# tangxyw/RecAlgorithm

Hardware: NVIDIA H100
Metric: ctr_fwd_bwd_samples_per_sec (higher is better)
Workload: dtype f32

## Files before the change

### recalgorithm_b200/csrc/c_api.cu

```cuda
#include <stdarg.h>
#include <string.h>

#include <atomic>

#include "ctr_common.cuh"

namespace ctr {
static thread_local char g_err[512] = "";
static std::atomic<long long> g_launches{0};

void set_error(const char* fmt, ...) {
  va_list ap;
  va_start(ap, fmt);
  vsnprintf(g_err, sizeof(g_err), fmt, ap);
  va_end(ap);
}
void count_launch(int n) { g_launches.fetch_add(n, std::memory_order_relaxed); }

int sm_count() {
  static int cached[64] = {0};
  int dev = 0;
  if (cudaGetDevice(&dev) != cudaSuccess || dev < 0 || dev >= 64) return 132;
  if (cached[dev] == 0) {
    int n = 0;
    if (cudaDeviceGetAttribute(&n, cudaDevAttrMultiProcessorCount, dev) != cudaSuccess || n <= 0) n = 132;
    cached[dev] = n;
  }
  return cached[dev];
}
}

extern "C" {
const char* ctr_last_error(void) { return ctr::g_err; }
int ctr_version(void) { return 1; }
int64_t ctr_kernel_launches(void) { return ctr::g_launches.load(); }

int ctr_enable_peer_access(int peer_device) {
  int dev = 0;
  CTR_CUDA(cudaGetDevice(&dev));
  if (peer_device == dev) return CTR_OK;
  int can = 0;
  CTR_CUDA(cudaDeviceCanAccessPeer(&can, dev, peer_device));
  if (!can) {
    ctr::set_error("ctr_enable_peer_access: device %d cannot access device %d over P2P", dev, peer_device);
    return CTR_ERR_UNSUPPORTED;
  }
  cudaError_t e = cudaDeviceEnablePeerAccess(peer_device, 0);
  if (e == cudaErrorPeerAccessAlreadyEnabled) { cudaGetLastError(); return CTR_OK; }
  if (e != cudaSuccess) {
    ctr::set_error("cudaDeviceEnablePeerAccess(%d) failed: %s", peer_device, cudaGetErrorString(e));
    return CTR_ERR_CUDA;
  }
  return CTR_OK;
}

int ctr_peer_alloc(int64_t bytes, void** ptr) {
  CTR_REQUIRE(ptr != nullptr && bytes > 0, "ctr_peer_alloc: bad arguments");
  CTR_CUDA(cudaMalloc(ptr, (size_t)bytes));
  return CTR_OK;
}
int ctr_peer_free(void* ptr) {
  if (ptr) CTR_CUDA(cudaFree(ptr));
  return CTR_OK;
}
int ctr_ipc_export(void* ptr, unsigned char* handle64) {
  CTR_REQUIRE(ptr && handle64, "ctr_ipc_export: null argument");
  static_assert(sizeof(cudaIpcMemHandle_t) == 64, "CUDA IPC handle is 64 bytes");
  cudaIpcMemHandle_t h;
  CTR_CUDA(cudaIpcGetMemHandle(&h, ptr));
  memcpy(handle64, &h, 64);
  return CTR_OK;
}
int ctr_ipc_import(const unsigned char* handle64, void** ptr) {
  CTR_REQUIRE(ptr && handle64, "ctr_ipc_import: null argument");
  cudaIpcMemHandle_t h;
  memcpy(&h, handle64, 64);
  CTR_CUDA(cudaIpcOpenMemHandle(ptr, h, cudaIpcMemLazyEnablePeerAccess));
  return CTR_OK;
}
int ctr_ipc_close(void* ptr) {
  if (ptr) CTR_CUDA(cudaIpcCloseMemHandle(ptr));
  return CTR_OK;
}

int ctr_device_info(int* sm_count, int* cc_major, int* cc_minor) {
  int dev = 0;
  CTR_CUDA(cudaGetDevice(&dev));
  int v = 0;
  if (sm_count) { CTR_CUDA(cudaDeviceGetAttribute(&v, cudaDevAttrMultiProcessorCount, dev)); *sm_count = v; }
  if (cc_major) { CTR_CUDA(cudaDeviceGetAttribute(&v, cudaDevAttrComputeCapabilityMajor, dev)); *cc_major = v; }
  if (cc_minor) { CTR_CUDA(cudaDeviceGetAttribute(&v, cudaDevAttrComputeCapabilityMinor, dev)); *cc_minor = v; }
  return CTR_OK;
}
}
```

### recalgorithm_b200/csrc/ctr_common.cuh

```cuda
#pragma once
#include <cuda_runtime.h>
#include <stdint.h>
#include <stdio.h>

#include <type_traits>

#include "../../include/ctr_b200.h"

namespace ctr {

void set_error(const char* fmt, ...);
void count_launch(int n = 1);
int sm_count();

#define CTR_REQUIRE(cond, ...)                                   \
  do {                                                           \
    if (!(cond)) {                                               \
      ctr::set_error(__VA_ARGS__);                               \
      return CTR_ERR_INVALID_ARG;                                \
    }                                                            \
  } while (0)

#define CTR_UNSUPPORTED(cond, ...)                               \
  do {                                                           \
    if (cond) {                                                  \
      ctr::set_error(__VA_ARGS__);                               \
      return CTR_ERR_UNSUPPORTED;                                \
    }                                                            \
  } while (0)

#define CTR_CHECK_LAUNCH(name)                                                   \
  do {                                                                           \
    cudaError_t e__ = cudaGetLastError();                                        \
    if (e__ != cudaSuccess) {                                                    \
      ctr::set_error("%s: launch failed: %s", name, cudaGetErrorString(e__));    \
      return CTR_ERR_CUDA;                                                       \
    }                                                                            \
    ctr::count_launch();                                                         \
  } while (0)

#define CTR_CUDA(call)                                                           \
  do {                                                                           \
    cudaError_t e__ = (call);                                                    \
    if (e__ != cudaSuccess) {                                                    \
      ctr::set_error("%s failed: %s", #call, cudaGetErrorString(e__));           \
      return CTR_ERR_CUDA;                                                       \
    }                                                                            \
  } while (0)

__device__ __forceinline__ float warp_sum(float v) {
#pragma unroll
  for (int o = 16; o > 0; o >>= 1) v += __shfl_xor_sync(0xffffffffu, v, o);
  return v;
}

__device__ __forceinline__ float4 ldg_stream_f4(const float4* p) {
  float4 r;
  asm volatile("ld.global.nc.L1::no_allocate.v4.f32 {%0,%1,%2,%3}, [%4];"
               : "=f"(r.x), "=f"(r.y), "=f"(r.z), "=f"(r.w) : "l"(p));
  return r;
}
__device__ __forceinline__ void stg_stream_f4(float4* p, const float4& v) {
  asm volatile("st.global.cs.v4.f32 [%0], {%1,%2,%3,%4};" ::"l"(p), "f"(v.x), "f"(v.y), "f"(v.z), "f"(v.w)
               : "memory");
}
__device__ __forceinline__ long long ldg_stream_i64(const long long* p) {
  long long r;
  asm volatile("ld.global.nc.L1::no_allocate.s64 %0, [%1];" : "=l"(r) : "l"(p));
  return r;
}

static inline cudaStream_t as_stream(void* s) { return reinterpret_cast<cudaStream_t>(s); }
static inline bool aligned16(const void* p) { return (reinterpret_cast<uintptr_t>(p) & 15u) == 0; }

static inline int capped_grid(long long need, long long cap) { return (int)(need < cap ? need : cap); }

template <class... P, class... A>
int launch(const char* what, void (*k)(P...), dim3 grid, dim3 block, size_t smem, cudaStream_t st, const A&... args) {
  if (smem > 48 * 1024) CTR_CUDA(cudaFuncSetAttribute(k, cudaFuncAttributeMaxDynamicSharedMemorySize, (int)smem));
  k<<<grid, block, smem, st>>>(args...);
  CTR_CHECK_LAUNCH(what);
  return CTR_OK;
}

template <int MAX_PER_SM = 0, class... P, class... A>
int launch_resident(const char* what, void (*k)(P...), long long need, int block, size_t smem, cudaStream_t st,
                    const A&... args) {
  if (smem > 48 * 1024) CTR_CUDA(cudaFuncSetAttribute(k, cudaFuncAttributeMaxDynamicSharedMemorySize, (int)smem));
  int per_sm = 0;
  if (cudaOccupancyMaxActiveBlocksPerMultiprocessor(&per_sm, k, block, smem) != cudaSuccess || per_sm < 1) per_sm = 1;
  if (MAX_PER_SM > 0 && per_sm > MAX_PER_SM) per_sm = MAX_PER_SM;
  k<<<capped_grid(need, (long long)per_sm * sm_count()), block, smem, st>>>(args...);
  CTR_CHECK_LAUNCH(what);
  return CTR_OK;
}

template <int... Vs, class F>
int with_const(int v, F&& f) {
  int rc = CTR_OK;
  const bool hit = ((v == Vs && ((rc = f(std::integral_constant<int, Vs>{})), true)) || ...);
  if (!hit) {
    set_error("no kernel instantiation for %d", v);
    return CTR_ERR_INVALID_ARG;
  }
  return rc;
}
template <class F>
int with_lpr(int64_t D, F&& f) {
  return with_const<1, 2, 4, 8, 16, 32>((int)(D / 4), f);
}

}
```

### recalgorithm_b200/csrc/embed_fm2.cu

```cuda
#include "ctr_common.cuh"

namespace ctr {

__device__ __forceinline__ float4 f4_zero() { return make_float4(0.f, 0.f, 0.f, 0.f); }

struct PeerTables {
  const float4* base[8];
  int G, logG;
};

__device__ __forceinline__ long long load_id(const long long* p) { return ldg_stream_i64(p); }
__device__ __forceinline__ long long load_id(const int* p) {
  int r;
  asm volatile("ld.global.nc.L1::no_allocate.s32 %0, [%1];" : "=r"(r) : "l"(p));
  return (long long)r;
}
__device__ __forceinline__ float4 ld_peer_f4(const float4* p) {
  float4 r;
  asm volatile("ld.global.v4.f32 {%0,%1,%2,%3}, [%4];" : "=f"(r.x), "=f"(r.y), "=f"(r.z), "=f"(r.w) : "l"(p));
  return r;
}

template <int LPR, bool SH, int MINB, bool BI = false, typename IdT = long long, bool LIN = false, bool SEQ = false>
__global__ void __launch_bounds__(256, MINB)
embed_fm2_fwd_kernel(const float4* __restrict__ table, const PeerTables peers, const long long* __restrict__ row_off,
                     const IdT* __restrict__ ids, int B, int F, float4* __restrict__ tile,
                     float* __restrict__ fm2, long long* __restrict__ ids64_out,
                     const float4* __restrict__ wlin, float* __restrict__ lin) {
  constexpr int RPW = 32 / LPR;
  constexpr int UB = LPR < 8 ? LPR : 8;
  const unsigned full = 0xffffffffu;
  const int lane = threadIdx.x & 31;
  const int sub = lane / LPR;
  const int c = lane % LPR;
  const int warp0 = (blockIdx.x * blockDim.x + threadIdx.x) >> 5;
  const int nwarps = (gridDim.x * blockDim.x) >> 5;

  for (int b = warp0; b < B; b += nwarps) {
    float4 S = f4_zero(), Q = f4_zero();
    float lin_acc = 0.f;
    for (int f0 = 0; f0 < F; f0 += 32) {
      const int nf = min(32, F - f0);
      long long row = -1;
      if (lane < nf) {
        const long long id = load_id(ids + (size_t)b * F + f0 + lane);
        const long long lo = __ldg(row_off + (SEQ ? 0 : f0 + lane)), hi = __ldg(row_off + (SEQ ? 1 : f0 + lane + 1));
        row = (id >= 0 && id < hi - lo) ? lo + id : -1;
        if (sizeof(IdT) == 4 && ids64_out != nullptr) ids64_out[(size_t)b * F + f0 + lane] = id;
      }
#pragma unroll
      for (int it0 = 0; it0 < LPR; it0 += UB) {
        if (it0 * RPW >= nf) break;
        float4 v[UB];
        bool in[UB];
#pragma unroll
        for (int u = 0; u < UB; ++u) {
          const int fs = (it0 + u) * RPW + sub;
          const long long r = __shfl_sync(full, row, fs);
          in[u] = fs < nf;
          v[u] = f4_zero();
          if (in[u] && r >= 0) {
            if (SH) v[u] = ld_peer_f4(peers.base[r & (peers.G - 1)] + (size_t)(r >> peers.logG) * LPR + c);
            else v[u] = ldg_stream_f4(table + (size_t)r * LPR + c);
          }
        }
#pragma unroll
        for (int u = 0; u < UB; ++u) {
          S.x += v[u].x; S.y += v[u].y; S.z += v[u].z; S.w += v[u].w;
          Q.x = __fadd_rn(Q.x, __fmul_rn(v[u].x, v[u].x)); Q.y = __fadd_rn(Q.y, __fmul_rn(v[u].y, v[u].y));
          Q.z = __fadd_rn(Q.z, __fmul_rn(v[u].z, v[u].z)); Q.w = __fadd_rn(Q.w, __fmul_rn(v[u].w, v[u].w));
          if (tile != nullptr && in[u]) {
            const int fs = (it0 + u) * RPW + sub;
            stg_stream_f4(tile + ((size_t)b * F + f0 + fs) * LPR + c, v[u]);
          }
          if (LIN && in[u]) {
            const float4 w = __ldg(wlin + (size_t)(f0 + (it0 + u) * RPW + sub) * LPR + c);
            lin_acc += v[u].x * w.x + v[u].y * w.y + v[u].z * w.z + v[u].w * w.w;
          }
        }
      }
    }
    if (LIN) {
      lin_acc = warp_sum(lin_acc);
      if (lane == 0) lin[b] = lin_acc;
    }
    if (fm2 != nullptr) {
#pragma unroll
      for (int o = LPR; o < 32; o <<= 1) {
        S.x += __shfl_xor_sync(full, S.x, o); S.y += __shfl_xor_sync(full, S.y, o);
        S.z += __shfl_xor_sync(full, S.z, o); S.w += __shfl_xor_sync(full, S.w, o);
        Q.x += __shfl_xor_sync(full, Q.x, o); Q.y += __shfl_xor_sync(full, Q.y, o);
        Q.z += __shfl_xor_sync(full, Q.z, o); Q.w += __shfl_xor_sync(full, Q.w, o);
      }
      if (BI) {
        if (lane < LPR) {
          float4 r;
          r.x = 0.5f * __fsub_rn(__fmul_rn(S.x, S.x), Q.x); r.y = 0.5f * __fsub_rn(__fmul_rn(S.y, S.y), Q.y);
          r.z = 0.5f * __fsub_rn(__fmul_rn(S.z, S.z), Q.z); r.w = 0.5f * __fsub_rn(__fmul_rn(S.w, S.w), Q.w);
          reinterpret_cast<float4*>(fm2)[(size_t)b * LPR + c] = r;
        }
        continue;
      }
      float p = 0.5f * __fsub_rn(__fmul_rn(S.x, S.x), Q.x) + 0.5f * __fsub_rn(__fmul_rn(S.y, S.y), Q.y) +
                0.5f * __fsub_rn(__fmul_rn(S.z, S.z), Q.z) + 0.5f * __fsub_rn(__fmul_rn(S.w, S.w), Q.w);
#pragma unroll
      for (int o = 1; o < LPR; o <<= 1) p += __shfl_xor_sync(full, p, o);
      if (lane == 0) fm2[b] = p;
    }
  }
}

template <int LPR, int HOLD, bool BI = false>
__global__ void __launch_bounds__(256)
embed_fm2_bwd_kernel(const float4* __restrict__ tile, const float4* __restrict__ d_tile,
                     const float* __restrict__ d_fm2, int B, int F, float4* __restrict__ row_grads) {
  const unsigned full = 0xffffffffu;
  const int lane = threadIdx.x & 31;
  const int warp0 = (blockIdx.x * blockDim.x + threadIdx.x) >> 5;
  const int nwarps = (gridDim.x * blockDim.x) >> 5;
  const int n4 = F * LPR;

  for (int b = warp0; b < B; b += nwarps) {
    const float4* e_row = tile + (size_t)b * n4;
    float4* o_row = row_grads + (size_t)b * n4;
    const float4* dt_row = d_tile ? d_tile + (size_t)b * n4 : nullptr;
    float4 g4;
    if (BI) {
      g4 = __ldg(reinterpret_cast<const float4*>(d_fm2) + (size_t)b * LPR + lane % LPR);
    } else {
      const float g = d_fm2 ? __ldg(d_fm2 + b) : 0.f;
      g4 = make_float4(g, g, g, g);
    }
    float4 S = f4_zero();
    if (HOLD > 0) {
      constexpr int H = HOLD > 0 ? HOLD : 1;
      float4 e[H];
#pragma unroll
      for (int k = 0; k < H; ++k) {
        const int j = k * 32 + lane;
        e[k] = f4_zero();
        if (j < n4) e[k] = ldg_stream_f4(e_row + j);
      }
      float4 dt[H];
#pragma unroll
      for (int k = 0; k < H; ++k) {
        const int j = k * 32 + lane;
        dt[k] = f4_zero();
        if (dt_row != nullptr && j < n4) dt[k] = ldg_stream_f4(dt_row + j);
      }
#pragma unroll
      for (int k = 0; k < H; ++k) { S.x += e[k].x; S.y += e[k].y; S.z += e[k].z; S.w += e[k].w; }
#pragma unroll
      for (int o = LPR; o < 32; o <<= 1) {
        S.x += __shfl_xor_sync(full, S.x, o); S.y += __shfl_xor_sync(full, S.y, o);
        S.z += __shfl_xor_sync(full, S.z, o); S.w += __shfl_xor_sync(full, S.w, o);
      }
#pragma unroll
      for (int k = 0; k < H; ++k) {
        const int j = k * 32 + lane;
        if (j < n4) {
          float4 r;
          r.x = dt[k].x + g4.x * (S.x - e[k].x); r.y = dt[k].y + g4.y * (S.y - e[k].y);
          r.z = dt[k].z + g4.z * (S.z - e[k].z); r.w = dt[k].w + g4.w * (S.w - e[k].w);
          stg_stream_f4(o_row + j, r);
        }
      }
    } else {
      for (int j = lane; j < n4; j += 32) {
        const float4 v = __ldg(e_row + j);
        S.x += v.x; S.y += v.y; S.z += v.z; S.w += v.w;
      }
#pragma unroll
      for (int o = LPR; o < 32; o <<= 1) {
        S.x += __shfl_xor_sync(full, S.x, o); S.y += __shfl_xor_sync(full, S.y, o);
        S.z += __shfl_xor_sync(full, S.z, o); S.w += __shfl_xor_sync(full, S.w, o);
      }
      for (int j = lane; j < n4; j += 32) {
        const float4 v = __ldg(e_row + j);
        float4 r = dt_row ? ldg_stream_f4(dt_row + j) : f4_zero();
        r.x += g4.x * (S.x - v.x); r.y += g4.y * (S.y - v.y); r.z += g4.z * (S.z - v.z); r.w += g4.w * (S.w - v.w);
        stg_stream_f4(o_row + j, r);
      }
    }
  }
}

template <int LPR, int HOLD>
__global__ void __launch_bounds__(256, 2)
embed_fm2_lin_bwd_kernel(const float4* __restrict__ tile, const float4* __restrict__ wlin, const float* __restrict__ d_fm2,
                         const float* __restrict__ d_lin, int B, int F, float4* __restrict__ row_grads,
                         float4* __restrict__ d_wlin) {
  extern __shared__ float4 s_lin[];
  const unsigned full = 0xffffffffu;
  const int lane = threadIdx.x & 31;
  const int warp0 = (blockIdx.x * blockDim.x + threadIdx.x) >> 5;
  const int nwarps = (gridDim.x * blockDim.x) >> 5;
  const int n4 = F * LPR;
  float4* s_w = s_lin;
  float4* s_dw = s_lin + n4;
  for (int j = threadIdx.x; j < n4; j += blockDim.x) { s_w[j] = __ldg(wlin + j); s_dw[j] = f4_zero(); }
  __syncthreads();
  float4 acc[HOLD];
#pragma unroll
  for (int k = 0; k < HOLD; ++k) acc[k] = f4_zero();
  for (int b = warp0; b < B; b += nwarps) {
    const float4* e_row = tile + (size_t)b * n4;
    float4* o_row = row_grads + (size_t)b * n4;
    const float g = d_fm2 ? __ldg(d_fm2 + b) : 0.f;
    const float gl = d_lin ? __ldg(d_lin + b) : 0.f;
    float4 e[HOLD];
#pragma unroll
    for (int k = 0; k < HOLD; ++k) {
      const int j = k * 32 + lane;
      e[k] = f4_zero();
      if (j < n4) e[k] = ldg_stream_f4(e_row + j);
    }
    float4 S = f4_zero();
#pragma unroll
    for (int k = 0; k < HOLD; ++k) { S.x += e[k].x; S.y += e[k].y; S.z += e[k].z; S.w += e[k].w; }
#pragma unroll
    for (int o = LPR; o < 32; o <<= 1) {
      S.x += __shfl_xor_sync(full, S.x, o); S.y += __shfl_xor_sync(full, S.y, o);
      S.z += __shfl_xor_sync(full, S.z, o); S.w += __shfl_xor_sync(full, S.w, o);
    }
#pragma unroll
    for (int k = 0; k < HOLD; ++k) {
      const int j = k * 32 + lane;
      if (j < n4) {
        const float4 w = s_w[j];
        float4 r;
        r.x = gl * w.x + g * (S.x - e[k].x); r.y = gl * w.y + g * (S.y - e[k].y);
        r.z = gl * w.z + g * (S.z - e[k].z); r.w = gl * w.w + g * (S.w - e[k].w);
        stg_stream_f4(o_row + j, r);
        acc[k].x += gl * e[k].x; acc[k].y += gl * e[k].y; acc[k].z += gl * e[k].z; acc[k].w += gl * e[k].w;
      }
    }
  }
#pragma unroll
  for (int k = 0; k < HOLD; ++k) {
    const int j = k * 32 + lane;
    if (j < n4) {
      atomicAdd(&s_dw[j].x, acc[k].x); atomicAdd(&s_dw[j].y, acc[k].y);
      atomicAdd(&s_dw[j].z, acc[k].z); atomicAdd(&s_dw[j].w, acc[k].w);
    }
  }
  __syncthreads();
  for (int j = threadIdx.x; j < n4; j += blockDim.x) atomicAdd(d_wlin + j, s_dw[j]);
}

template <int LPR>
__global__ void __launch_bounds__(256)
embed_scatter_add_kernel(float4* __restrict__ grad_table, const long long* __restrict__ row_off,
                         const long long* __restrict__ ids, const float4* __restrict__ row_grads, int B, int F) {
  const size_t total = (size_t)B * F * LPR;
  for (size_t t = (size_t)blockIdx.x * blockDim.x + threadIdx.x; t < total; t += (size_t)gridDim.x * blockDim.x) {
    const int c = (int)(t % LPR);
    const size_t bf = t / LPR;
    const int f = (int)(bf % F);
    const long long id = __ldg(ids + bf);
    const long long lo = __ldg(row_off + f), hi = __ldg(row_off + f + 1);
    if (id >= 0 && id < hi - lo) {
      const float4 g = ldg_stream_f4(row_grads + t);
      atomicAdd(grad_table + (size_t)(lo + id) * LPR + c, g);
    }
  }
}

__global__ void __launch_bounds__(256)
bag_lookup_fwd_kernel(const float* __restrict__ table, long long V, int D, const long long* __restrict__ ids,
                      const long long* __restrict__ offsets, int B, float* __restrict__ out, long long out_stride,
                      int G) {
  const int tid = blockIdx.x * blockDim.x + threadIdx.x;
  const int gl = threadIdx.x % G;
  const int nthreads = gridDim.x * blockDim.x;
  for (int b = tid / G; b < B; b += nthreads / G) {
    const long long s = __ldg(offsets + b), e = __ldg(offsets + b + 1);
    float acc[8];
#pragma unroll
    for (int k = 0; k < 8; ++k) acc[k] = 0.f;
    int n = 0;
    for (long long i = s; i < e; ++i) {
      const long long id = __ldg(ids + i);
      if (id >= 0 && id < V) {
        ++n;
#pragma unroll
        for (int k = 0; k < 8; ++k) {
          const int dd = k * G + gl;
          if (dd < D) acc[k] += __ldg(table + (size_t)id * D + dd);
        }
      }
    }
#pragma unroll
    for (int k = 0; k < 8; ++k) {
      const int dd = k * G + gl;
      if (dd < D) out[(size_t)b * out_stride + dd] = n > 0 ? acc[k] / (float)n : 0.f;
    }
  }
}

__global__ void __launch_bounds__(256)
bag_lookup_bwd_kernel(const float* __restrict__ d_out, long long out_stride, long long V, int D,
                      const long long* __restrict__ ids, const long long* __restrict__ offsets, int B,
                      float* __restrict__ row_grads, int G) {
  const int tid = blockIdx.x * blockDim.x + threadIdx.x;
  const int gl = threadIdx.x % G;
  const int nthreads = gridDim.x * blockDim.x;
  for (int b = tid / G; b < B; b += nthreads / G) {
    const long long s = __ldg(offsets + b), e = __ldg(offsets + b + 1);
    int n = 0;
    for (long long i = s; i < e; ++i) {
      const long long id = __ldg(ids + i);
      n += (id >= 0 && id < V);
    }
    for (long long i = s; i < e; ++i) {
      const long long id = __ldg(ids + i);
      const bool ok = id >= 0 && id < V;
      for (int dd = gl; dd < D; dd += G) {
        const float g = __ldg(d_out + (size_t)b * out_stride + dd);
        row_grads[(size_t)i * D + dd] = ok ? g / (float)n : 0.f;
      }
    }
  }
}

__global__ void __launch_bounds__(256)
first_order_fwd_kernel(const float* __restrict__ w, const long long* __restrict__ row_off,
                       const long long* __restrict__ ids, int B, int F, float bias, float* __restrict__ out) {
  const int lane = threadIdx.x & 31;
  const int warp0 = (blockIdx.x * blockDim.x + threadIdx.x) >> 5;
  const int nwarps = (gridDim.x * blockDim.x) >> 5;
  for (int b = warp0; b < B; b += nwarps) {
    float acc = 0.f;
    for (int f = lane; f < F; f += 32) {
      const long long id = ldg_stream_i64(ids + (size_t)b * F + f);
      const long long lo = __ldg(row_off + f), hi = __ldg(row_off + f + 1);
      if (id >= 0 && id < hi - lo) acc += __ldg(w + lo + id);
    }
    acc = warp_sum(acc);
    if (lane == 0) out[b] = acc + bias;
  }
}

template <int LPR, typename IdT>
static int launch_fwd(const float* table, const PeerTables* peers, const int64_t* off, const IdT* ids, int64_t B,
                      int64_t F, float* tile, float* fm2, int64_t* ids64_out, cudaStream_t st) {
  PeerTables none = {};
  const PeerTables& pt = peers ? *peers : none;
  auto go = [&](auto k) {
    return launch_resident("ctr_embed_fm2_fwd", k, (B + 7) / 8, 256, 0, st, reinterpret_cast<const float4*>(table), pt,
                           reinterpret_cast<const long long*>(off), ids, (int)B, (int)F, reinterpret_cast<float4*>(tile), fm2,
                           reinterpret_cast<long long*>(ids64_out), nullptr, nullptr);
  };
  return peers != nullptr ? go(embed_fm2_fwd_kernel<LPR, true, 1, false, IdT>) : go(embed_fm2_fwd_kernel<LPR, false, 4, false, IdT>);
}

template <int LPR, int HOLD, bool BI = false>
static int launch_bwd(const float* tile, const float* d_tile, const float* d_fm2, int64_t B, int64_t F,
                      float* row_grads, cudaStream_t st) {
  return launch_resident("ctr_embed_fm2_bwd", embed_fm2_bwd_kernel<LPR, HOLD, BI>, (B + 7) / 8, 256, 0, st,
                         reinterpret_cast<const float4*>(tile), reinterpret_cast<const float4*>(d_tile), d_fm2, (int)B, (int)F,
                         reinterpret_cast<float4*>(row_grads));
}

template <int LPR, bool BI = false>
static int dispatch_bwd(const float* tile, const float* d_tile, const float* d_fm2, int64_t B, int64_t F,
                        float* row_grads, cudaStream_t st) {
  const int64_t per_lane = (F * LPR + 31) / 32;
  if (per_lane <= 4) return launch_bwd<LPR, 4, BI>(tile, d_tile, d_fm2, B, F, row_grads, st);
  if (per_lane <= 8) return launch_bwd<LPR, 8, BI>(tile, d_tile, d_fm2, B, F, row_grads, st);
  if (per_lane <= 12) return launch_bwd<LPR, 12, BI>(tile, d_tile, d_fm2, B, F, row_grads, st);
  return launch_bwd<LPR, 0, BI>(tile, d_tile, d_fm2, B, F, row_grads, st);
}

template <int LPR>
static int launch_fwd_bi(const float* table, const int64_t* off, const int64_t* ids, int64_t B, int64_t F, float* tile,
                         float* bi, cudaStream_t st) {
  return launch_resident("ctr_embed_bi_fwd", embed_fm2_fwd_kernel<LPR, false, 4, true>, (B + 7) / 8, 256, 0, st,
                         reinterpret_cast<const float4*>(table), PeerTables{}, reinterpret_cast<const long long*>(off),
                         reinterpret_cast<const long long*>(ids), (int)B, (int)F, reinterpret_cast<float4*>(tile), bi, nullptr,
                         nullptr, nullptr);
}

static int check_bfd(const char* fn, int64_t B, int64_t F, int64_t D) {
  CTR_REQUIRE(B >= 0 && F >= 1 && D >= 1, "%s: bad sizes B=%lld F=%lld D=%lld", fn, (long long)B, (long long)F,
              (long long)D);
  CTR_REQUIRE(B <= 0x7fffffffLL / 8 && F <= 65536, "%s: B=%lld / F=%lld too large", fn, (long long)B, (long long)F);
  CTR_UNSUPPORTED(D % 4 != 0 || D > 128 || (D & (D - 1)) != 0,
                  "%s: D=%lld unsupported by the fused 128-bit path (need a power of two in 4..128); "
                  "use ctr_bag_lookup_* for other widths", fn, (long long)D);
  return CTR_OK;
}

template <typename IdT>
static int dispatch_fwd(const float* table, const PeerTables* peers, const int64_t* off, const IdT* ids, int64_t B,
                        int64_t F, int64_t D, float* tile, float* fm2, int64_t* ids64_out, cudaStream_t st) {
  return with_lpr(D, [&](auto LPR) { return launch_fwd<LPR>(table, peers, off, ids, B, F, tile, fm2, ids64_out, st); });
}

static int fill_peers(const char* fn, PeerTables& peers, const float* const* shard_ptrs, int64_t G) {
  CTR_REQUIRE(G >= 1 && G <= 8 && (G & (G - 1)) == 0, "%s: G=%lld must be a power of two <= 8", fn, (long long)G);
  peers = PeerTables{};
  peers.G = (int)G;
  while ((1 << peers.logG) < G) ++peers.logG;
  for (int r = 0; r < G; ++r) {
    CTR_REQUIRE(shard_ptrs[r] != nullptr && aligned16(shard_ptrs[r]), "%s: shard %d null/unaligned", fn, r);
    peers.base[r] = reinterpret_cast<const float4*>(shard_ptrs[r]);
  }
  return CTR_OK;
}

}

using namespace ctr;

extern "C" int ctr_embed_fm2_fwd(const float* table, const int64_t* field_row_offset, const int64_t* ids,
                                 int64_t B, int64_t F, int64_t D, float* tile, float* fm2, void* stream) {
  int rc = check_bfd("ctr_embed_fm2_fwd", B, F, D);
  if (rc) return rc;
  CTR_REQUIRE(table && field_row_offset && ids, "ctr_embed_fm2_fwd: null table/field_row_offset/ids");
  CTR_REQUIRE(tile || fm2, "ctr_embed_fm2_fwd: both outputs are NULL");
  CTR_REQUIRE(aligned16(table) && aligned16(tile), "ctr_embed_fm2_fwd: table and tile must be 16-byte aligned");
  if (B == 0) return CTR_OK;
  cudaStream_t st = as_stream(stream);
  return dispatch_fwd(table, nullptr, field_row_offset, reinterpret_cast<const long long*>(ids), B, F, D, tile, fm2, nullptr, st);
}

extern "C" int ctr_embed_fm2_fwd_ids32(const float* table, const int64_t* field_row_offset, const int32_t* ids, int64_t B,
                                       int64_t F, int64_t D, float* tile, float* fm2, int64_t* ids64_out, void* stream) {
  int rc = check_bfd("ctr_embed_fm2_fwd_ids32", B, F, D);
  if (rc) return rc;
  CTR_REQUIRE(table && field_row_offset && ids, "ctr_embed_fm2_fwd_ids32: null table/field_row_offset/ids");
  CTR_REQUIRE(tile || fm2, "ctr_embed_fm2_fwd_ids32: both outputs are NULL");
  CTR_REQUIRE(aligned16(table) && aligned16(tile), "ctr_embed_fm2_fwd_ids32: table and tile must be 16-byte aligned");
  if (B == 0) return CTR_OK;
  return dispatch_fwd(table, nullptr, field_row_offset, reinterpret_cast<const int*>(ids), B, F, D, tile, fm2, ids64_out,
                      as_stream(stream));
}

extern "C" int ctr_embed_fm2_fwd_sharded(const float* const* shard_ptrs, int64_t G, const int64_t* field_row_offset,
                                         const int64_t* ids, int64_t B, int64_t F, int64_t D, float* tile, float* fm2,
                                         void* stream) {
  int rc = check_bfd("ctr_embed_fm2_fwd_sharded", B, F, D);
  if (rc) return rc;
  CTR_REQUIRE(shard_ptrs && field_row_offset && ids, "ctr_embed_fm2_fwd_sharded: null shard_ptrs/field_row_offset/ids");
  CTR_REQUIRE(tile || fm2, "ctr_embed_fm2_fwd_sharded: both outputs are NULL");
  PeerTables peers;
  rc = fill_peers("ctr_embed_fm2_fwd_sharded", peers, shard_ptrs, G);
  if (rc) return rc;
  CTR_REQUIRE(aligned16(tile), "ctr_embed_fm2_fwd_sharded: tile must be 16-byte aligned");
  if (B == 0) return CTR_OK;
  return dispatch_fwd(nullptr, &peers, field_row_offset, reinterpret_cast<const long long*>(ids), B, F, D, tile, fm2, nullptr,
                      as_stream(stream));
}

extern "C" int ctr_embed_fm2_fwd_sharded_ids32(const float* const* shard_ptrs, int64_t G, const int64_t* field_row_offset,
                                               const int32_t* ids, int64_t B, int64_t F, int64_t D, float* tile, float* fm2,
                                               int64_t* ids64_out, void* stream) {
  int rc = check_bfd("ctr_embed_fm2_fwd_sharded_ids32", B, F, D);
  if (rc) return rc;
  CTR_REQUIRE(shard_ptrs && field_row_offset && ids, "ctr_embed_fm2_fwd_sharded_ids32: null shard_ptrs/field_row_offset/ids");
  CTR_REQUIRE(tile || fm2, "ctr_embed_fm2_fwd_sharded_ids32: both outputs are NULL");
  PeerTables peers;
  rc = fill_peers("ctr_embed_fm2_fwd_sharded_ids32", peers, shard_ptrs, G);
  if (rc) return rc;
  CTR_REQUIRE(aligned16(tile), "ctr_embed_fm2_fwd_sharded_ids32: tile must be 16-byte aligned");
  if (B == 0) return CTR_OK;
  return dispatch_fwd(nullptr, &peers, field_row_offset, reinterpret_cast<const int*>(ids), B, F, D, tile, fm2, ids64_out,
                      as_stream(stream));
}

extern "C" int ctr_embed_fm2_bwd(const float* tile, const float* d_tile, const float* d_fm2, int64_t B, int64_t F,
                                 int64_t D, float* row_grads, void* stream) {
  int rc = check_bfd("ctr_embed_fm2_bwd", B, F, D);
  if (rc) return rc;
  CTR_REQUIRE(tile && row_grads, "ctr_embed_fm2_bwd: null tile/row_grads");
  CTR_REQUIRE(aligned16(tile) && aligned16(d_tile) && aligned16(row_grads),
              "ctr_embed_fm2_bwd: tile, d_tile and row_grads must be 16-byte aligned");
  if (B == 0) return CTR_OK;
  cudaStream_t st = as_stream(stream);
  return with_lpr(D, [&](auto LPR) { return dispatch_bwd<LPR>(tile, d_tile, d_fm2, B, F, row_grads, st); });
}

extern "C" int ctr_embed_scatter_add(float* grad_table, const int64_t* field_row_offset, const int64_t* ids,
                                     const float* row_grads, int64_t B, int64_t F, int64_t D, void* stream) {
  int rc = check_bfd("ctr_embed_scatter_add", B, F, D);
  if (rc) return rc;
  CTR_REQUIRE(grad_table && field_row_offset && ids && row_grads, "ctr_embed_scatter_add: null argument");
  CTR_REQUIRE(aligned16(grad_table) && aligned16(row_grads), "ctr_embed_scatter_add: buffers must be 16-byte aligned");
  if (B == 0) return CTR_OK;
  cudaStream_t st = as_stream(stream);
  const long long total = (long long)B * F * (D / 4);
  const int grid = capped_grid((total + 255) / 256, (long long)sm_count() * 16);
  return with_lpr(D, [&](auto LPR) {
    return launch("ctr_embed_scatter_add", embed_scatter_add_kernel<LPR>, grid, 256, 0, st, reinterpret_cast<float4*>(grad_table),
                  reinterpret_cast<const long long*>(field_row_offset), reinterpret_cast<const long long*>(ids),
                  reinterpret_cast<const float4*>(row_grads), (int)B, (int)F);
  });
}

static int bag_group(int64_t D) {
  int G = 1;
  while (G < D && G < 32) G <<= 1;
  return G;
}

extern "C" int ctr_bag_lookup_fwd(const float* table, int64_t V, int64_t D, const int64_t* ids,
                                  const int64_t* offsets, int64_t B, float* out, int64_t out_stride, void* stream) {
  CTR_REQUIRE(table && offsets && out, "ctr_bag_lookup_fwd: null argument");
  CTR_REQUIRE(B >= 0 && V >= 0 && D >= 1 && out_stride >= D, "ctr_bag_lookup_fwd: bad sizes");
  CTR_UNSUPPORTED(D > 256, "ctr_bag_lookup_fwd: D=%lld > 256", (long long)D);
  if (B == 0) return CTR_OK;
  const int G = bag_group(D);
  return launch("ctr_bag_lookup_fwd", bag_lookup_fwd_kernel, capped_grid(((long long)B * G + 255) / 256, (long long)sm_count() * 16),
                256, 0, as_stream(stream), table, V, (int)D, reinterpret_cast<const long long*>(ids),
                reinterpret_cast<const long long*>(offsets), (int)B, out, out_stride, G);
}

extern "C" int ctr_bag_lookup_bwd(const float* d_out, int64_t out_stride, int64_t V, int64_t D, const int64_t* ids,
                                  const int64_t* offsets, int64_t B, float* row_grads, void* stream) {
  CTR_REQUIRE(d_out && offsets, "ctr_bag_lookup_bwd: null argument");
  CTR_REQUIRE(B >= 0 && V >= 0 && D >= 1 && out_stride >= D, "ctr_bag_lookup_bwd: bad sizes");
  CTR_UNSUPPORTED(D > 256, "ctr_bag_lookup_bwd: D=%lld > 256", (long long)D);
  if (B == 0) return CTR_OK;
  const int G = bag_group(D);
  return launch("ctr_bag_lookup_bwd", bag_lookup_bwd_kernel, capped_grid(((long long)B * G + 255) / 256, (long long)sm_count() * 16),
                256, 0, as_stream(stream), d_out, out_stride, V, (int)D, reinterpret_cast<const long long*>(ids),
                reinterpret_cast<const long long*>(offsets), (int)B, row_grads, G);
}

extern "C" int ctr_first_order_fwd(const float* w, const int64_t* field_row_offset, const int64_t* ids, int64_t B,
                                   int64_t F, float bias, float* out, void* stream) {
  CTR_REQUIRE(w && field_row_offset && ids && out, "ctr_first_order_fwd: null argument");
  CTR_REQUIRE(B >= 0 && F >= 1 && B <= 0x7fffffffLL / 8 && F <= 65536, "ctr_first_order_fwd: bad sizes");
  if (B == 0) return CTR_OK;
  return launch("ctr_first_order_fwd", first_order_fwd_kernel, capped_grid((B + 7) / 8, (long long)sm_count() * 8), 256, 0,
                as_stream(stream), w, reinterpret_cast<const long long*>(field_row_offset), reinterpret_cast<const long long*>(ids),
                (int)B, (int)F, bias, out);
}

extern "C" int ctr_embed_bi_fwd(const float* table, const int64_t* field_row_offset, const int64_t* ids, int64_t B, int64_t F,
                                int64_t D, float* tile, float* bi, void* stream) {
  int rc = check_bfd("ctr_embed_bi_fwd", B, F, D);
  if (rc) return rc;
  CTR_REQUIRE(table && field_row_offset && ids && bi, "ctr_embed_bi_fwd: null table/field_row_offset/ids/bi");
  CTR_REQUIRE(aligned16(table) && aligned16(tile) && aligned16(bi), "ctr_embed_bi_fwd: table, tile and bi must be 16-byte aligned");
  if (B == 0) return CTR_OK;
  cudaStream_t st = as_stream(stream);
  return with_lpr(D, [&](auto LPR) { return launch_fwd_bi<LPR>(table, field_row_offset, ids, B, F, tile, bi, st); });
}

extern "C" int ctr_embed_bi_bwd(const float* tile, const float* d_tile, const float* d_bi, int64_t B, int64_t F, int64_t D,
                                float* row_grads, void* stream) {
  int rc = check_bfd("ctr_embed_bi_bwd", B, F, D);
  if (rc) return rc;
  CTR_REQUIRE(tile && d_bi && row_grads, "ctr_embed_bi_bwd: null tile/d_bi/row_grads");
  CTR_REQUIRE(aligned16(tile) && aligned16(d_tile) && aligned16(d_bi) && aligned16(row_grads),
              "ctr_embed_bi_bwd: tile, d_tile, d_bi and row_grads must be 16-byte aligned");
  if (B == 0) return CTR_OK;
  cudaStream_t st = as_stream(stream);
  return with_lpr(D, [&](auto LPR) { return dispatch_bwd<LPR, true>(tile, d_tile, d_bi, B, F, row_grads, st); });
}

template <int LPR, typename IdT>
static int launch_fwd_lin(const float* table, const PeerTables* peers, const int64_t* off, const IdT* ids, int64_t B, int64_t F,
                          float* tile, float* fm2, int64_t* ids64_out, const float* wlin, float* lin, cudaStream_t st) {
  auto go = [&](auto k, const float4* tb, const PeerTables& pt) {
    return launch_resident("ctr_embed_fm2_lin_fwd", k, (B + 7) / 8, 256, 0, st, tb, pt, reinterpret_cast<const long long*>(off),
                           ids, (int)B, (int)F, reinterpret_cast<float4*>(tile), fm2, reinterpret_cast<long long*>(ids64_out),
                           reinterpret_cast<const float4*>(wlin), lin);
  };
  if (peers != nullptr) return go(embed_fm2_fwd_kernel<LPR, true, 1, false, IdT, true>, nullptr, *peers);
  return go(embed_fm2_fwd_kernel<LPR, false, 3, false, IdT, true>, reinterpret_cast<const float4*>(table), PeerTables{});
}

template <typename IdT>
static int dispatch_fwd_lin(const float* table, const PeerTables* peers, const int64_t* off, const IdT* ids, int64_t B, int64_t F,
                            int64_t D, float* tile, float* fm2, int64_t* ids64_out, const float* wlin, float* lin, cudaStream_t st) {
  return with_lpr(D, [&](auto LPR) { return launch_fwd_lin<LPR>(table, peers, off, ids, B, F, tile, fm2, ids64_out, wlin, lin, st); });
}

extern "C" int ctr_embed_fm2_lin_fwd(const float* table, const int64_t* field_row_offset, const void* ids, int ids_are_int32,
                                     int64_t B, int64_t F, int64_t D, const float* wlin, float* tile, float* fm2, float* lin,
                                     int64_t* ids64_out, void* stream) {
  int rc = check_bfd("ctr_embed_fm2_lin_fwd", B, F, D);
  if (rc) return rc;
  CTR_REQUIRE(table && field_row_offset && ids && wlin && lin, "ctr_embed_fm2_lin_fwd: null table/field_row_offset/ids/wlin/lin");
  CTR_REQUIRE(aligned16(table) && aligned16(tile) && aligned16(wlin), "ctr_embed_fm2_lin_fwd: table, tile and wlin must be 16-byte aligned");
  if (B == 0) return CTR_OK;
  cudaStream_t st = as_stream(stream);
  if (ids_are_int32)
    return dispatch_fwd_lin(table, nullptr, field_row_offset, reinterpret_cast<const int*>(ids), B, F, D, tile, fm2, ids64_out, wlin, lin, st);
  return dispatch_fwd_lin(table, nullptr, field_row_offset, reinterpret_cast<const long long*>(ids), B, F, D, tile, fm2, nullptr, wlin, lin, st);
}

extern "C" int ctr_embed_fm2_lin_fwd_sharded(const float* const* shard_ptrs, int64_t G, const int64_t* field_row_offset,
                                             const void* ids, int ids_are_int32, int64_t B, int64_t F, int64_t D, const float* wlin,
                                             float* tile, float* fm2, float* lin, int64_t* ids64_out, void* stream) {
  int rc = check_bfd("ctr_embed_fm2_lin_fwd_sharded", B, F, D);
  if (rc) return rc;
  CTR_REQUIRE(shard_ptrs && field_row_offset && ids && wlin && lin, "ctr_embed_fm2_lin_fwd_sharded: null argument");
  PeerTables peers;
  rc = fill_peers("ctr_embed_fm2_lin_fwd_sharded", peers, shard_ptrs, G);
  if (rc) return rc;
  CTR_REQUIRE(aligned16(tile) && aligned16(wlin), "ctr_embed_fm2_lin_fwd_sharded: tile and wlin must be 16-byte aligned");
  if (B == 0) return CTR_OK;
  cudaStream_t st = as_stream(stream);
  if (ids_are_int32)
    return dispatch_fwd_lin(nullptr, &peers, field_row_offset, reinterpret_cast<const int*>(ids), B, F, D, tile, fm2, ids64_out, wlin, lin, st);
  return dispatch_fwd_lin(nullptr, &peers, field_row_offset, reinterpret_cast<const long long*>(ids), B, F, D, tile, fm2, nullptr, wlin, lin, st);
}

template <int LPR, int HOLD>
static int launch_lin_bwd(const float* tile, const float* wlin, const float* d_fm2, const float* d_lin, int64_t B, int64_t F,
                          float* row_grads, float* d_wlin, cudaStream_t st) {
  return launch_resident("ctr_embed_fm2_lin_bwd", embed_fm2_lin_bwd_kernel<LPR, HOLD>, (B + 7) / 8, 256,
                         sizeof(float4) * 2 * (size_t)F * LPR, st, reinterpret_cast<const float4*>(tile),
                         reinterpret_cast<const float4*>(wlin), d_fm2, d_lin, (int)B, (int)F, reinterpret_cast<float4*>(row_grads),
                         reinterpret_cast<float4*>(d_wlin));
}

template <int LPR>
static int dispatch_lin_bwd(const float* tile, const float* wlin, const float* d_fm2, const float* d_lin, int64_t B, int64_t F,
                            float* row_grads, float* d_wlin, cudaStream_t st) {
  const int64_t per_lane = (F * LPR + 31) / 32;
  if (per_lane <= 4) return launch_lin_bwd<LPR, 4>(tile, wlin, d_fm2, d_lin, B, F, row_grads, d_wlin, st);
  if (per_lane <= 8) return launch_lin_bwd<LPR, 8>(tile, wlin, d_fm2, d_lin, B, F, row_grads, d_wlin, st);
  if (per_lane <= 12) return launch_lin_bwd<LPR, 12>(tile, wlin, d_fm2, d_lin, B, F, row_grads, d_wlin, st);
  set_error("ctr_embed_fm2_lin_bwd: F*D = %lld exceeds the register-resident limit of 1536", (long long)(F * LPR * 4));
  return CTR_ERR_UNSUPPORTED;
}

extern "C" int ctr_embed_fm2_lin_bwd(const float* tile, const float* wlin, const float* d_fm2, const float* d_lin, int64_t B,
                                     int64_t F, int64_t D, float* row_grads, float* d_wlin, void* stream) {
  int rc = check_bfd("ctr_embed_fm2_lin_bwd", B, F, D);
  if (rc) return rc;
  CTR_REQUIRE(tile && wlin && row_grads && d_wlin, "ctr_embed_fm2_lin_bwd: null tile/wlin/row_grads/d_wlin");
  CTR_REQUIRE(aligned16(tile) && aligned16(wlin) && aligned16(row_grads) && aligned16(d_wlin),
              "ctr_embed_fm2_lin_bwd: buffers must be 16-byte aligned");
  cudaStream_t st = as_stream(stream);
  CTR_CUDA(cudaMemsetAsync(d_wlin, 0, sizeof(float) * F * D, st));
  if (B == 0) return CTR_OK;
  return with_lpr(D, [&](auto LPR) { return dispatch_lin_bwd<LPR>(tile, wlin, d_fm2, d_lin, B, F, row_grads, d_wlin, st); });
}

template <int LPR>
static int launch_seq(const float* table, const int64_t* range2, const int64_t* ids, int64_t B, int64_t T, float* out, cudaStream_t st) {
  return launch_resident("ctr_embed_seq_fwd", embed_fm2_fwd_kernel<LPR, false, 4, false, long long, false, true>, (B + 7) / 8, 256,
                         0, st, reinterpret_cast<const float4*>(table), PeerTables{}, reinterpret_cast<const long long*>(range2),
                         reinterpret_cast<const long long*>(ids), (int)B, (int)T, reinterpret_cast<float4*>(out), nullptr, nullptr,
                         nullptr, nullptr);
}

extern "C" int ctr_embed_seq_fwd(const float* table, const int64_t* row_range, const int64_t* ids, int64_t B, int64_t T, int64_t D,
                                 float* out, void* stream) {
  int rc = check_bfd("ctr_embed_seq_fwd", B, T > 0 ? T : 1, D);
  if (rc) return rc;
  CTR_REQUIRE(table && row_range && out && (ids || B * T == 0), "ctr_embed_seq_fwd: null argument");
  CTR_REQUIRE(aligned16(table) && aligned16(out), "ctr_embed_seq_fwd: table and out must be 16-byte aligned");
  if (B == 0 || T == 0) return CTR_OK;
  cudaStream_t st = as_stream(stream);
  return with_lpr(D, [&](auto LPR) { return launch_seq<LPR>(table, row_range, ids, B, T, out, st); });
}
```

Measured before the change: 107.0 million.

## Keep tail of forward tile in L2 and consume it first in backward

The forward embedding kernel now stores the last rows of the tile (those with b >= keep_from, sized to about 7/8 of L2) with an evict_last cache policy. The ids and table reads are marked evict_first so they do not push that tile out. The backward kernel walks batch rows in reverse, so it reads the still-resident tail of the tile first, and it marks its tile and d_tile reads evict_first. The goal is to turn part of the backward tile reread into L2 hits instead of HBM traffic, at the cost of extra policy instructions and some dependence on how much L2 is actually free.

```diff
diff --git a/recalgorithm_b200/csrc/c_api.cu b/recalgorithm_b200/csrc/c_api.cu
--- a/recalgorithm_b200/csrc/c_api.cu
+++ b/recalgorithm_b200/csrc/c_api.cu
@@ -24,6 +24,18 @@
   if (cached[dev] == 0) {
     int n = 0;
     if (cudaDeviceGetAttribute(&n, cudaDevAttrMultiProcessorCount, dev) != cudaSuccess || n <= 0) n = 132;
+    cached[dev] = n;
+  }
+  return cached[dev];
+}
+
+long long l2_bytes() {
+  static int cached[64] = {0};
+  int dev = 0;
+  if (cudaGetDevice(&dev) != cudaSuccess || dev < 0 || dev >= 64) return 50LL << 20;
+  if (cached[dev] == 0) {
+    int n = 0;
+    if (cudaDeviceGetAttribute(&n, cudaDevAttrL2CacheSize, dev) != cudaSuccess || n <= 0) n = 50 << 20;
     cached[dev] = n;
   }
   return cached[dev];
diff --git a/recalgorithm_b200/csrc/ctr_common.cuh b/recalgorithm_b200/csrc/ctr_common.cuh
--- a/recalgorithm_b200/csrc/ctr_common.cuh
+++ b/recalgorithm_b200/csrc/ctr_common.cuh
@@ -12,6 +12,7 @@
 void set_error(const char* fmt, ...);
 void count_launch(int n = 1);
 int sm_count();
+long long l2_bytes();
 
 #define CTR_REQUIRE(cond, ...)                                   \
   do {                                                           \
@@ -83,14 +84,19 @@
   return CTR_OK;
 }
 
+template <int MAX_PER_SM = 0, class... P>
+int resident_grid(void (*k)(P...), long long need, int block, size_t smem) {
+  int per_sm = 0;
+  if (cudaOccupancyMaxActiveBlocksPerMultiprocessor(&per_sm, k, block, smem) != cudaSuccess || per_sm < 1) per_sm = 1;
+  if (MAX_PER_SM > 0 && per_sm > MAX_PER_SM) per_sm = MAX_PER_SM;
+  return capped_grid(need, (long long)per_sm * sm_count());
+}
+
 template <int MAX_PER_SM = 0, class... P, class... A>
 int launch_resident(const char* what, void (*k)(P...), long long need, int block, size_t smem, cudaStream_t st,
                     const A&... args) {
   if (smem > 48 * 1024) CTR_CUDA(cudaFuncSetAttribute(k, cudaFuncAttributeMaxDynamicSharedMemorySize, (int)smem));
-  int per_sm = 0;
-  if (cudaOccupancyMaxActiveBlocksPerMultiprocessor(&per_sm, k, block, smem) != cudaSuccess || per_sm < 1) per_sm = 1;
-  if (MAX_PER_SM > 0 && per_sm > MAX_PER_SM) per_sm = MAX_PER_SM;
-  k<<<capped_grid(need, (long long)per_sm * sm_count()), block, smem, st>>>(args...);
+  k<<<resident_grid<MAX_PER_SM>(k, need, block, smem), block, smem, st>>>(args...);
   CTR_CHECK_LAUNCH(what);
   return CTR_OK;
 }
diff --git a/recalgorithm_b200/csrc/embed_fm2.cu b/recalgorithm_b200/csrc/embed_fm2.cu
--- a/recalgorithm_b200/csrc/embed_fm2.cu
+++ b/recalgorithm_b200/csrc/embed_fm2.cu
@@ -15,6 +15,34 @@
   asm volatile("ld.global.nc.L1::no_allocate.s32 %0, [%1];" : "=r"(r) : "l"(p));
   return (long long)r;
 }
+
+__device__ __forceinline__ uint64_t l2_evict_first() {
+  uint64_t pol;
+  asm("createpolicy.fractional.L2::evict_first.b64 %0, 1.0;" : "=l"(pol));
+  return pol;
+}
+__device__ __forceinline__ long long load_id(const long long* p, uint64_t pol) {
+  long long r;
+  asm volatile("ld.global.nc.L1::no_allocate.L2::cache_hint.s64 %0, [%1], %2;" : "=l"(r) : "l"(p), "l"(pol));
+  return r;
+}
+__device__ __forceinline__ long long load_id(const int* p, uint64_t pol) {
+  int r;
+  asm volatile("ld.global.nc.L1::no_allocate.L2::cache_hint.s32 %0, [%1], %2;" : "=r"(r) : "l"(p), "l"(pol));
+  return (long long)r;
+}
+__device__ __forceinline__ float4 ldg_stream_f4(const float4* p, uint64_t pol) {
+  float4 r;
+  asm volatile("ld.global.nc.L1::no_allocate.L2::cache_hint.v4.f32 {%0,%1,%2,%3}, [%4], %5;"
+               : "=f"(r.x), "=f"(r.y), "=f"(r.z), "=f"(r.w) : "l"(p), "l"(pol));
+  return r;
+}
+__device__ __forceinline__ void stg_tile_f4(float4* p, const float4& v, bool keep) {
+  asm volatile("{\n\t.reg .pred k;\n\t.reg .b64 pol;\n\tsetp.ne.b32 k, %5, 0;\n\t"
+               "createpolicy.fractional.L2::evict_last.b64 pol, 1.0;\n\t"
+               "@k st.global.L2::cache_hint.v4.f32 [%0], {%1,%2,%3,%4}, pol;\n\t@!k st.global.cs.v4.f32 [%0], {%1,%2,%3,%4};\n\t}"
+               ::"l"(p), "f"(v.x), "f"(v.y), "f"(v.z), "f"(v.w), "r"((int)keep) : "memory");
+}
 __device__ __forceinline__ float4 ld_peer_f4(const float4* p) {
   float4 r;
   asm volatile("ld.global.v4.f32 {%0,%1,%2,%3}, [%4];" : "=f"(r.x), "=f"(r.y), "=f"(r.z), "=f"(r.w) : "l"(p));
@@ -26,7 +54,8 @@
 embed_fm2_fwd_kernel(const float4* __restrict__ table, const PeerTables peers, const long long* __restrict__ row_off,
                      const IdT* __restrict__ ids, int B, int F, float4* __restrict__ tile,
                      float* __restrict__ fm2, long long* __restrict__ ids64_out,
-                     const float4* __restrict__ wlin, float* __restrict__ lin) {
+                     const float4* __restrict__ wlin, float* __restrict__ lin, int keep_from) {
+  constexpr bool HANDOFF = !SH && !LIN && !SEQ;
   constexpr int RPW = 32 / LPR;
   constexpr int UB = LPR < 8 ? LPR : 8;
   const unsigned full = 0xffffffffu;
@@ -43,7 +72,7 @@
       const int nf = min(32, F - f0);
       long long row = -1;
       if (lane < nf) {
-        const long long id = load_id(ids + (size_t)b * F + f0 + lane);
+        const long long id = HANDOFF ? load_id(ids + (size_t)b * F + f0 + lane, l2_evict_first()) : load_id(ids + (size_t)b * F + f0 + lane);
         const long long lo = __ldg(row_off + (SEQ ? 0 : f0 + lane)), hi = __ldg(row_off + (SEQ ? 1 : f0 + lane + 1));
         row = (id >= 0 && id < hi - lo) ? lo + id : -1;
         if (sizeof(IdT) == 4 && ids64_out != nullptr) ids64_out[(size_t)b * F + f0 + lane] = id;
@@ -61,6 +90,7 @@
           v[u] = f4_zero();
           if (in[u] && r >= 0) {
             if (SH) v[u] = ld_peer_f4(peers.base[r & (peers.G - 1)] + (size_t)(r >> peers.logG) * LPR + c);
+            else if (HANDOFF) v[u] = ldg_stream_f4(table + (size_t)r * LPR + c, l2_evict_first());
             else v[u] = ldg_stream_f4(table + (size_t)r * LPR + c);
           }
         }
@@ -71,7 +101,8 @@
           Q.z = __fadd_rn(Q.z, __fmul_rn(v[u].z, v[u].z)); Q.w = __fadd_rn(Q.w, __fmul_rn(v[u].w, v[u].w));
           if (tile != nullptr && in[u]) {
             const int fs = (it0 + u) * RPW + sub;
-            stg_stream_f4(tile + ((size_t)b * F + f0 + fs) * LPR + c, v[u]);
+            if (HANDOFF) stg_tile_f4(tile + ((size_t)b * F + f0 + fs) * LPR + c, v[u], b >= keep_from);
+            else stg_stream_f4(tile + ((size_t)b * F + f0 + fs) * LPR + c, v[u]);
           }
           if (LIN && in[u]) {
             const float4 w = __ldg(wlin + (size_t)(f0 + (it0 + u) * RPW + sub) * LPR + c);
@@ -119,8 +150,10 @@
   const int warp0 = (blockIdx.x * blockDim.x + threadIdx.x) >> 5;
   const int nwarps = (gridDim.x * blockDim.x) >> 5;
   const int n4 = F * LPR;
-
-  for (int b = warp0; b < B; b += nwarps) {
+  const uint64_t once = l2_evict_first();
+
+  for (int i = warp0; i < B; i += nwarps) {
+    const int b = B - 1 - i;
     const float4* e_row = tile + (size_t)b * n4;
     float4* o_row = row_grads + (size_t)b * n4;
     const float4* dt_row = d_tile ? d_tile + (size_t)b * n4 : nullptr;
@@ -139,14 +172,14 @@
       for (int k = 0; k < H; ++k) {
         const int j = k * 32 + lane;
         e[k] = f4_zero();
-        if (j < n4) e[k] = ldg_stream_f4(e_row + j);
+        if (j < n4) e[k] = ldg_stream_f4(e_row + j, once);
       }
       float4 dt[H];
 #pragma unroll
       for (int k = 0; k < H; ++k) {
         const int j = k * 32 + lane;
         dt[k] = f4_zero();
-        if (dt_row != nullptr && j < n4) dt[k] = ldg_stream_f4(dt_row + j);
+        if (dt_row != nullptr && j < n4) dt[k] = ldg_stream_f4(dt_row + j, once);
       }
 #pragma unroll
       for (int k = 0; k < H; ++k) { S.x += e[k].x; S.y += e[k].y; S.z += e[k].z; S.w += e[k].w; }
@@ -177,7 +210,7 @@
       }
       for (int j = lane; j < n4; j += 32) {
         const float4 v = __ldg(e_row + j);
-        float4 r = dt_row ? ldg_stream_f4(dt_row + j) : f4_zero();
+        float4 r = dt_row ? ldg_stream_f4(dt_row + j, once) : f4_zero();
         r.x += g4.x * (S.x - v.x); r.y += g4.y * (S.y - v.y); r.z += g4.z * (S.z - v.z); r.w += g4.w * (S.w - v.w);
         stg_stream_f4(o_row + j, r);
       }
@@ -341,15 +374,22 @@
   }
 }
 
+static int l2_keep_from(int64_t B, int64_t F, int LPR, int grid) {
+  if ((F * LPR + 31) / 32 > 12) return (int)B;
+  const long long per_round = (long long)grid * 8, round_bytes = per_round * F * LPR * 16;
+  return (int)(B - l2_bytes() * 7 / 8 / round_bytes * per_round);
+}
+
 template <int LPR, typename IdT>
 static int launch_fwd(const float* table, const PeerTables* peers, const int64_t* off, const IdT* ids, int64_t B,
                       int64_t F, float* tile, float* fm2, int64_t* ids64_out, cudaStream_t st) {
   PeerTables none = {};
   const PeerTables& pt = peers ? *peers : none;
   auto go = [&](auto k) {
-    return launch_resident("ctr_embed_fm2_fwd", k, (B + 7) / 8, 256, 0, st, reinterpret_cast<const float4*>(table), pt,
-                           reinterpret_cast<const long long*>(off), ids, (int)B, (int)F, reinterpret_cast<float4*>(tile), fm2,
-                           reinterpret_cast<long long*>(ids64_out), nullptr, nullptr);
+    const int grid = resident_grid(k, (B + 7) / 8, 256, 0);
+    return launch("ctr_embed_fm2_fwd", k, grid, 256, 0, st, reinterpret_cast<const float4*>(table), pt,
+                  reinterpret_cast<const long long*>(off), ids, (int)B, (int)F, reinterpret_cast<float4*>(tile), fm2,
+                  reinterpret_cast<long long*>(ids64_out), nullptr, nullptr, l2_keep_from(B, F, LPR, grid));
   };
   return peers != nullptr ? go(embed_fm2_fwd_kernel<LPR, true, 1, false, IdT>) : go(embed_fm2_fwd_kernel<LPR, false, 4, false, IdT>);
 }
@@ -375,10 +415,11 @@
 template <int LPR>
 static int launch_fwd_bi(const float* table, const int64_t* off, const int64_t* ids, int64_t B, int64_t F, float* tile,
                          float* bi, cudaStream_t st) {
-  return launch_resident("ctr_embed_bi_fwd", embed_fm2_fwd_kernel<LPR, false, 4, true>, (B + 7) / 8, 256, 0, st,
-                         reinterpret_cast<const float4*>(table), PeerTables{}, reinterpret_cast<const long long*>(off),
-                         reinterpret_cast<const long long*>(ids), (int)B, (int)F, reinterpret_cast<float4*>(tile), bi, nullptr,
-                         nullptr, nullptr);
+  auto k = embed_fm2_fwd_kernel<LPR, false, 4, true>;
+  const int grid = resident_grid(k, (B + 7) / 8, 256, 0);
+  return launch("ctr_embed_bi_fwd", k, grid, 256, 0, st, reinterpret_cast<const float4*>(table), PeerTables{},
+                reinterpret_cast<const long long*>(off), reinterpret_cast<const long long*>(ids), (int)B, (int)F,
+                reinterpret_cast<float4*>(tile), bi, nullptr, nullptr, nullptr, l2_keep_from(B, F, LPR, grid));
 }
 
 static int check_bfd(const char* fn, int64_t B, int64_t F, int64_t D) {
@@ -567,7 +608,7 @@
   auto go = [&](auto k, const float4* tb, const PeerTables& pt) {
     return launch_resident("ctr_embed_fm2_lin_fwd", k, (B + 7) / 8, 256, 0, st, tb, pt, reinterpret_cast<const long long*>(off),
                            ids, (int)B, (int)F, reinterpret_cast<float4*>(tile), fm2, reinterpret_cast<long long*>(ids64_out),
-                           reinterpret_cast<const float4*>(wlin), lin);
+                           reinterpret_cast<const float4*>(wlin), lin, (int)B);
   };
   if (peers != nullptr) return go(embed_fm2_fwd_kernel<LPR, true, 1, false, IdT, true>, nullptr, *peers);
   return go(embed_fm2_fwd_kernel<LPR, false, 3, false, IdT, true>, reinterpret_cast<const float4*>(table), PeerTables{});
@@ -648,7 +689,7 @@
   return launch_resident("ctr_embed_seq_fwd", embed_fm2_fwd_kernel<LPR, false, 4, false, long long, false, true>, (B + 7) / 8, 256,
                          0, st, reinterpret_cast<const float4*>(table), PeerTables{}, reinterpret_cast<const long long*>(range2),
                          reinterpret_cast<const long long*>(ids), (int)B, (int)T, reinterpret_cast<float4*>(out), nullptr, nullptr,
-                         nullptr, nullptr);
+                         nullptr, nullptr, (int)B);
 }
 
 extern "C" int ctr_embed_seq_fwd(const float* table, const int64_t* row_range, const int64_t* ids, int64_t B, int64_t T, int64_t D,
```

Measured after the change: 108.2 million (median of 6 runs). +1.1%, better.
